# leoelm/Bayesian_inference_for_NN

Measured on AMD Instinct MI355X. Metric: posterior samples/sec (grad-steps/sec) on MLP 784->200->10, batch 1024, higher is better.
Workload: dtype f32; 1 GPU; SGLD, MLP 784->200->10 (D=159010), synthetic MNIST-shaped 48000x784 fp32 resident in HBM, batch 1024 (last batch of an epoch 896), 1 chain per GPU, device-resident run replayed from hipGraphs; seed=2024, parallelism=independent chains x1 (replicas only, no data-path collective)

## Files before the change

bayesian_inference_for_nn_amd/csrc/pyz_api.hip:

```cpp

#include <algorithm>
#include <cmath>
#include <cstring>

#include "pyz_common.h"
#include "pyz_fused.h"
#include "pyz_gemm.h"
#include "pyz_gemm_ring.h"
#include "pyz_hmc_fused.h"
#include "pyz_hmc_multi.h"
#include "pyz_kernels.h"
#include "pyz_rng.h"

namespace {

inline hipStream_t as_stream(void *s) { return reinterpret_cast<hipStream_t>(s); }
inline int cdiv(long long a, long long b) { return (int)((a + b - 1) / b); }

int ensure_bytes(void **ptr, size_t *cap, size_t need, pyz_mlp *m) {
  if (*cap >= need) return PYZ_OK;
  if (*ptr) PYZ_HIP(hipFree(*ptr));
  *ptr = nullptr;
  *cap = 0;
  PYZ_HIP(hipMalloc(ptr, need));
// ... 189 lines not shown
      g.out_pstride = (long long)m->max_batch * K;
      g.aux = m->act[l - 1];
      g.aux_pstride = (long long)m->max_batch * K;
      g.act = m->acts[l - 1];
      g.vec = (N % 8 == 0) && (m->w_off[l] % 4 == 0) && (P == 1 || theta_ps % 4 == 0) && aligned16(theta) ? 1 : 0;
      g.ctl = ctl;
      pyz_launch_bwd_data(g, grid_batch, P, st);
    }
    DenseArgs g{};
    g.K = K;
    g.N = N;
    if (l == 0) {
      g.in = x;
      g.in_pstride = 0;
      g.row_idx = row_idx;
    } else {
      g.in = m->act[l - 1];
      g.in_pstride = (long long)m->max_batch * K;
    }
    g.lda = K;
    g.aux = m->delta[l];
    g.aux_pstride = (long long)m->max_batch * N;
    g.out = grad;
    g.out_pstride = m->D;
    g.w_off = m->w_off[l];
    g.ctl = ctl;
    if (grad_sq) pyz_launch_bwd_weight_sq(g, grad_sq, grid_batch, st);
    else pyz_launch_bwd_weight(g, grid_batch, P, st);
  }
}

inline bool can_fuse(const pyz_mlp *m) { return m->dims[m->L] <= 32; }

void launch_head(pyz_mlp *m, const float *theta, long long theta_ps, int P, const float *x, const void *y,
                 const int32_t *row_idx, int grid_batch, const StepCtl *ctl, bool want_delta, hipStream_t st,
                 const StepCtl *gate = nullptr, int gate_mod = 0, int k_split = 0) {
  const int l = m->L - 1;
  HeadArgs g{};
  g.gate = gate;
  g.gate_mod = gate_mod;
  if (k_split > 1) {
    g.hparts = static_cast<const float *>(full(m)->x.fwd_part);
    g.n_hparts = k_split;
    g.hpart_stride = (long long)m->max_batch * m->dims[l];
    g.bias_prev = theta + m->w_off[l - 1] + (long long)m->dims[l - 1] * m->dims[l];
    g.h_store = m->act[l - 1];
  }
  g.K = m->dims[l];
  g.N = m->dims[l + 1];
  if (l == 0) {
    g.hin = x;
    g.hin_pstride = 0;
    g.gather_hin = 1;
  } else {
    g.hin = m->act[l - 1];
    g.hin_pstride = (long long)m->max_batch * g.K;
    g.gather_hin = 0;
  }
  g.lda = g.K;
  g.row_idx = row_idx;
  g.theta = theta;
  g.theta_pstride = theta_ps;
  g.w_off = m->w_off[l];
  g.loss = m->loss;
  g.act_last = m->acts[l];
  g.act_prev = l > 0 ? m->acts[l - 1] : PYZ_ACT_LINEAR;
  g.vec = (g.K % 8 == 0) && aligned16(g.hin) ? 1 : 0;
  g.y = y;
  g.out_last = m->act[l];
  g.delta_last = want_delta ? m->delta[l] : nullptr;
  g.delta_prev = (want_delta && l > 0) ? m->delta[l - 1] : nullptr;
  g.last_pstride = (long long)m->max_batch * g.N;
  g.prev_pstride = (long long)m->max_batch * g.K;
  g.part = m->part;
  g.ctl = ctl;
  g.wt = pyz_wt_for(P);
  if (m->pend_on && ctl == m->ctl) {
    g.init = m->pend;
    g.init_on = 1;
    m->pend_on = false;
  }
  static const int rows_on = pyz_env_int("PYZ_HEAD_ROWS", 1);
  const int UT = g.K <= 64 ? 1 : g.K <= 256 ? 4 : g.K <= 512 ? 8 : g.K <= 1024 ? 16 : 0;
  const int NP = g.N <= 4 ? 4 : g.N <= 8 ? 8 : g.N <= 12 ? 12 : g.N <= 16 ? 16 : g.N <= 24 ? 24 : 32;
  if (rows_on && UT && UT * NP <= 128) {
    g.nblk = grid_batch;
    m->cur_nblk = g.nblk;
    static const int rw_rows = pyz_env_int("PYZ_HEAD_RW_ROWS", 32768);
    const int RW = (long long)P * grid_batch >= rw_rows ? 4 : 1;
    const dim3 grid((unsigned)cdiv(cdiv(grid_batch, RW), 4), P), block(256);
    if (g.n_hparts > 0) {
      if (NP == 4) PYZ_LAUNCH((k_head_rows<4, 4, 1, true>), grid, block, 0, st, g);
      else if (NP == 8) PYZ_LAUNCH((k_head_rows<4, 8, 1, true>), grid, block, 0, st, g);
      else if (NP == 12) PYZ_LAUNCH((k_head_rows<4, 12, 1, true>), grid, block, 0, st, g);
      else PYZ_LAUNCH((k_head_rows<4, 16, 1, true>), grid, block, 0, st, g);
      return;
    }
#define PYZ_HEAD_ROWS_CASE(U, C)                                                               \
  if (UT == U && NP == C) {                                                                    \
    if (RW == 4) PYZ_LAUNCH((k_head_rows<U, C, 4>), grid, block, 0, st, g);                     \
    else PYZ_LAUNCH((k_head_rows<U, C, 1>), grid, block, 0, st, g);                            \
    return;                                                                                    \
  }
    PYZ_HEAD_ROWS_CASE(1, 4) PYZ_HEAD_ROWS_CASE(1, 8) PYZ_HEAD_ROWS_CASE(1, 12) PYZ_HEAD_ROWS_CASE(1, 16)
    PYZ_HEAD_ROWS_CASE(1, 24) PYZ_HEAD_ROWS_CASE(1, 32)
    PYZ_HEAD_ROWS_CASE(4, 4) PYZ_HEAD_ROWS_CASE(4, 8) PYZ_HEAD_ROWS_CASE(4, 12) PYZ_HEAD_ROWS_CASE(4, 16)
    PYZ_HEAD_ROWS_CASE(4, 24) PYZ_HEAD_ROWS_CASE(4, 32)
    PYZ_HEAD_ROWS_CASE(8, 4) PYZ_HEAD_ROWS_CASE(8, 8) PYZ_HEAD_ROWS_CASE(8, 12) PYZ_HEAD_ROWS_CASE(8, 16)
    PYZ_HEAD_ROWS_CASE(16, 4) PYZ_HEAD_ROWS_CASE(16, 8)
#undef PYZ_HEAD_ROWS_CASE
  }
  g.nblk = cdiv(grid_batch, 32);
  m->cur_nblk = g.nblk;
  static const int head_waves = pyz_env_int("PYZ_HEAD_WAVES", 8) >= 8 ? 8 : 4;
  PYZ_LAUNCH(k_head, dim3(g.nblk, P), dim3(64 * head_waves), head_waves * 4096 + 2 * 32 * 33 * 4 + 64, st, g);
}

void launch_bwd_data_hidden(pyz_mlp *m, const float *theta, long long theta_ps, int P, int grid_batch,
                            const StepCtl *ctl, hipStream_t st) {
  for (int l = m->L - 2; l >= 1; --l) {
    const int K = m->dims[l], N = m->dims[l + 1];
    DenseArgs g{};
    g.K = K;
    g.N = N;
    g.in = m->delta[l];
    g.in_pstride = (long long)m->max_batch * N;
    g.lda = N;
    g.theta = theta;
    g.theta_pstride = theta_ps;
    g.w_off = m->w_off[l];
    g.out = m->delta[l - 1];
    g.out_pstride = (long long)m->max_batch * K;
    g.aux = m->act[l - 1];
    g.aux_pstride = (long long)m->max_batch * K;
    g.act = m->acts[l - 1];
    g.vec = (N % 8 == 0) && (m->w_off[l] % 4 == 0) && (P == 1 || theta_ps % 4 == 0) && aligned16(theta) ? 1 : 0;
    g.ctl = ctl;
    pyz_launch_bwd_data(g, grid_batch, P, st);
  }
}

inline int wgrad_tiles(const pyz_mlp *m) {
  int tiles = 0;
  for (int l = 0; l < m->L; ++l) tiles += ((m->dims[l] + 1 + 31) / 32) * ((m->dims[l + 1] + 31) / 32);
  return tiles;
}

int wgrad_layers(pyz_mlp *m, int P, const float *x, const int32_t *row_idx, const StepCtl *ctl, WgradArgs &a,
// ... 68 lines not shown
  static const int on = pyz_env_int("PYZ_BATCH_AHEAD", 1);
  if (!on || !can_fuse(m) || m->L <= 1 || row_idx == nullptr) return false;
  return on == 2 || wgrad_tiles(m) + 24 <= pyz_cu_count();
}

PrepArgs prep_args(pyz_mlp *m, const float *x, const int32_t *row_idx, int grid_batch, long long row_stride, int dst_slot) {
  PrepArgs p{};
  p.src = x;
  p.dst = batch_buf(m, dst_slot);
  p.row_idx = row_idx;
  p.tab_bs = m->tab_bs;
  p.row_stride = row_stride;
  p.K = p.lda = m->dims[0];
  p.fwd_tiles_n = (m->dims[1] + 31) / 32;
  p.fwd_tiles = ((grid_batch + 31) / 32) * p.fwd_tiles_n;
  return p;
}

int ksplit_for(pyz_mlp *m, const float *theta, long long theta_ps, int P, const float *xc, int grid_batch, const StepCtl *ctl) {
  const int ks_env = pyz_env_int("PYZ_FWD_KSPLIT", 0);
  if (ks_env < 2 || ks_env > 8 || m->L != 2 || P != 1) return 0;
  const int UT = m->dims[1] <= 64 ? 1 : m->dims[1] <= 256 ? 4 : 0, NPc = m->dims[2];
  if (!UT || NPc > 16 || !pyz_env_int("PYZ_HEAD_ROWS", 1)) return 0;
  DenseArgs g = forward_args(m, 0, theta, theta_ps, xc, nullptr, ctl, nullptr);
  if (!pyz_fwd_ring_ksplit_ok(g, grid_batch, P)) return 0;
  if ((long long)((grid_batch + 31) / 32) * ks_env > 2 * pyz_cu_count()) return 0;
  const size_t need = sizeof(float) * (size_t)ks_env * m->max_batch * m->dims[1];
  if (!full(m)->x.fwd_part || full(m)->x.fwd_part_cap < need) return 0;
  return ks_env;
}

void launch_loss_backward(pyz_mlp *m, const float *theta, long long theta_ps, int P, const float *x, const void *y,
                          const int32_t *row_idx, int grid_batch, const StepCtl *ctl, bool want_grad, WgradArgs &upd,
                          hipStream_t st, int ahead_slot = -1, AdamArgs *adam = nullptr) {
  if (can_fuse(m)) {
    if (ahead_slot >= 0) {
      const float *xc = batch_buf(m, ahead_slot);
      const int ks = ksplit_for(m, theta, theta_ps, P, xc, grid_batch, ctl);
      if (ks > 1) {
        DenseArgs g = forward_args(m, 0, theta, theta_ps, xc, nullptr, ctl, nullptr);
        g.wt = pyz_wt_for(P);
        g.k_split = ks;
        g.part_out = static_cast<float *>(full(m)->x.fwd_part);
        g.part_stride = (long long)m->max_batch * g.N;
        pyz_launch_fwd_ring_ksplit(g, grid_batch, st);
      } else {
        launch_forward(m, theta, theta_ps, P, xc, nullptr, grid_batch, ctl, st, nullptr, m->L - 1);
      }
      launch_head(m, theta, theta_ps, P, x, y, row_idx, grid_batch, ctl, want_grad, st, nullptr, 0, ks);
      launch_bwd_data_hidden(m, theta, theta_ps, P, grid_batch, ctl, st);
      launch_wgrad_all(m, P, x, row_idx, grid_batch, ctl, upd, st, xc);
      return;
    }
    static const int use_xb = pyz_env_int("PYZ_GATHER_COPY", 1);
    float *xb = (use_xb && want_grad && row_idx && m->L > 1) ? m->xb : nullptr;
    launch_forward(m, theta, theta_ps, P, x, row_idx, grid_batch, ctl, st, xb, m->L - 1);
    launch_head(m, theta, theta_ps, P, x, y, row_idx, grid_batch, ctl, want_grad, st);
    if (want_grad) {
      launch_bwd_data_hidden(m, theta, theta_ps, P, grid_batch, ctl, st);
      if (adam) launch_wgrad_adam(m, x, row_idx, grid_batch, ctl, *adam, st, xb);
      else launch_wgrad_all(m, P, x, row_idx, grid_batch, ctl, upd, st, xb);
    }
    return;
  }
  flush_ctl(m, st);
  launch_forward(m, theta, theta_ps, P, x, row_idx, grid_batch, ctl, st);
  launch_loss(m, P, y, row_idx, grid_batch, ctl, want_grad, st);
  m->cur_nblk = loss_nblk(m, grid_batch);
  if (want_grad) launch_backward(m, theta, theta_ps, P, x, row_idx, grid_batch, ctl, upd.grad, st, adam ? m->grad2 : nullptr);
}

int check_loss_combo(const pyz_mlp *m) {
  const int last = m->acts[m->L - 1];
  if (m->loss == PYZ_LOSS_SCCE && last != PYZ_ACT_SOFTMAX)
    return pyz_fail(PYZ_E_INVALID, "SparseCategoricalCrossentropy needs a softmax last layer");
  if (m->loss == PYZ_LOSS_MSE && last == PYZ_ACT_SOFTMAX)
    return pyz_fail(PYZ_E_INVALID, "MeanSquaredError on a softmax last layer is not supported");
  return PYZ_OK;
}

AdamScal adam_scalars(float lr, double beta_1, double beta_2, long long epoch, float denom_eps, float decay) {
  AdamScal a;
// ... 61 lines not shown
    long long widest = 0;
    for (int l = 0; l <= n_layers; ++l) widest = std::max<long long>(widest, m->dims[l]);
    if ((long long)max_batch * widest * 4 >= (1LL << 31) || off * 4 >= (1LL << 31)) {
      delete m;
      return pyz_fail(PYZ_E_INVALID, "max_batch x widest layer, or the parameter vector, exceeds 2 GiB");
    }
  }
  auto fail = [&](int rc) {
    pyz_mlp_destroy(m);
    return rc;
  };
  for (int l = 0; l < n_layers; ++l) {
    const size_t bytes = sizeof(float) * (size_t)max_particles * max_batch * m->dims[l + 1] + 64;
    if (hipMalloc((void **)&m->act[l], bytes) != hipSuccess || hipMalloc((void **)&m->delta[l], bytes) != hipSuccess)
      return fail(pyz_fail(PYZ_E_OOM, "workspace allocation of %zu bytes failed", bytes));
    m->ws_bytes += 2 * bytes;
  }
  {
    const size_t bytes = 2 * sizeof(float) * (size_t)max_batch * m->dims[0] + 64;
    if (hipMalloc((void **)&m->xb, bytes) != hipSuccess) return fail(pyz_fail(PYZ_E_OOM, "workspace allocation of %zu bytes failed", bytes));
    m->ws_bytes += bytes;
  }
  if (hipMalloc((void **)&m->nonfinite, 64) != hipSuccess || hipMemset(m->nonfinite, 0, 64) != hipSuccess)
    return fail(pyz_fail(PYZ_E_OOM, "counter allocation failed"));
  if (hipMalloc((void **)&m->ctl, 2 * sizeof(StepCtl)) != hipSuccess) return fail(pyz_fail(PYZ_E_OOM, "ctl allocation failed"));
  if (hipMemset(m->ctl, 0, 2 * sizeof(StepCtl)) != hipSuccess) return fail(pyz_fail(PYZ_E_HIP, "ctl memset failed"));
  const size_t scal = sizeof(float) * (size_t)(max_particles * 16 + 64);
  if (hipMalloc((void **)&m->scal, scal) != hipSuccess) return fail(pyz_fail(PYZ_E_OOM, "scalar allocation failed"));
  m->ws_bytes += scal;
  {
    const int rc = need_part(m, (size_t)max_particles * max_batch + 8);
    if (rc != PYZ_OK) return fail(rc);
  }
  if (m->L == 2 && m->dims[1] > 192 && m->dims[1] <= 200 && pyz_env_int("PYZ_FWD_KSPLIT", 0) >= 2) {
    const int rc = ensure_bytes(&m->x.fwd_part, &m->x.fwd_part_cap, sizeof(float) * (size_t)8 * max_batch * m->dims[1], m);
    if (rc != PYZ_OK) return fail(rc);
  }
  {
    const int gs_lds = (int)pyz_svgd_gs_lds_bytes();
    if (hipFuncSetAttribute(reinterpret_cast<const void *>(k_svgd_gs<false>), hipFuncAttributeMaxDynamicSharedMemorySize, gs_lds) != hipSuccess ||
        hipFuncSetAttribute(reinterpret_cast<const void *>(k_svgd_gs<true>), hipFuncAttributeMaxDynamicSharedMemorySize, gs_lds) != hipSuccess)
      return fail(pyz_fail(PYZ_E_HIP, "hipFuncSetAttribute(k_svgd_gs) failed"));
    if (hipFuncSetAttribute(reinterpret_cast<const void *>(k_svgd_gs_resident), hipFuncAttributeMaxDynamicSharedMemorySize,
                            (int)pyz_svgd_gs_res_lds_bytes()) != hipSuccess)
      return fail(pyz_fail(PYZ_E_HIP, "hipFuncSetAttribute(k_svgd_gs_resident) failed"));
    if (hipFuncSetAttribute(reinterpret_cast<const void *>(k_svgd_gs_resident2), hipFuncAttributeMaxDynamicSharedMemorySize,
                            (int)pyz_svgd_gs_res_lds_bytes()) != hipSuccess)
      return fail(pyz_fail(PYZ_E_HIP, "hipFuncSetAttribute(k_svgd_gs_resident2) failed"));
    const int gr_lds = (int)pyz_svgd_gram_lds_bytes();
    if (hipFuncSetAttribute(reinterpret_cast<const void *>(k_svgd_gram_tile<1, false>), hipFuncAttributeMaxDynamicSharedMemorySize, gr_lds) != hipSuccess ||
        hipFuncSetAttribute(reinterpret_cast<const void *>(k_svgd_gram_tile<2, false>), hipFuncAttributeMaxDynamicSharedMemorySize, gr_lds) != hipSuccess ||
        hipFuncSetAttribute(reinterpret_cast<const void *>(k_svgd_gram_tile<4, true>), hipFuncAttributeMaxDynamicSharedMemorySize, gr_lds) != hipSuccess)
      return fail(pyz_fail(PYZ_E_HIP, "hipFuncSetAttribute(k_svgd_gram_tile) failed"));
  }
  *out = m;
  return PYZ_OK;
}

int pyz_mlp_destroy(pyz_mlp *mm) {
  if (!mm) return PYZ_OK;
  pyz_mlp_full *m = full(mm);
  drop_graphs(m);
  if (m->x.hm_exec) (void)hipGraphExecDestroy(m->x.hm_exec);
  if (m->x.hm_graph) (void)hipGraphDestroy(m->x.hm_graph);
  for (int l = 0; l < PYZ_MAX_LAYERS; ++l) {
    if (m->act[l]) (void)hipFree(m->act[l]);
    if (m->delta[l]) (void)hipFree(m->delta[l]);
  }
  void *ptrs[] = {m->grad, m->grad2, m->qsave, m->part, m->x.part2, m->scal, m->ctl, m->tab_bs, m->xb, m->x.hm_buf, m->x.hm_res_buf, m->x.gs_res_buf, m->x.fwd_part, m->nonfinite};
  for (void *p : ptrs)
    if (p) (void)hipFree(p);
  if (m->x.tab_host) {
    (void)hipHostFree(m->x.tab_host);
    for (auto &e : m->x.tab_ev) (void)hipEventDestroy(e);
  }
  if (m->x.up_host) {
    (void)hipHostFree(m->x.up_host);
    for (auto &e : m->x.up_ev) (void)hipEventDestroy(e);
  }
  if (m->h_pinned) (void)hipHostFree(m->h_pinned);
  delete m;
  return PYZ_OK;
}

int64_t pyz_mlp_param_count(const pyz_mlp *m) { return m ? m->D : -1; }
int64_t pyz_mlp_workspace_bytes(const pyz_mlp *m) { return m ? (int64_t)m->ws_bytes : -1; }

int pyz_mlp_forward(pyz_mlp *m, const float *d_theta, int P, const float *d_x, const int32_t *d_row_idx, int batch,
                    float *d_out, void *stream) {
  int rc = check_call(m, P, batch);
  if (rc) return rc;
  if (!d_theta || !d_x || !d_out) return pyz_fail(PYZ_E_INVALID, "null device pointer");
  hipStream_t st = as_stream(stream);
  if ((rc = set_ctl(m, 0, batch, 0.0f, 0, 0, 0, st))) return rc;
  launch_forward(m, d_theta, m->D, P, d_x, d_row_idx, batch, m->ctl, st);
  const int C = m->dims[m->L];
  PYZ_LAUNCH(k_forward_finish, dim3(cdiv(batch, 256), P), dim3(256), 0, st, m->act[m->L - 1],
                     (long long)m->max_batch * C, C, m->acts[m->L - 1] == PYZ_ACT_SOFTMAX ? 1 : 0, batch, d_out);
  PYZ_LAUNCH_CHECK();
  return PYZ_OK;
}

// ... 197 lines not shown
    const bool ahead = chained && batch_ahead(m, row_idx);
    if (ahead) u.prep = prep_args(m, x, row_idx, grid_batch, row_stride, slot ^ 1);
    launch_loss_backward(m, w_cur, m->D, 1, x, y, row_idx, grid_batch, ctl, true, u, st, ahead ? slot : -1);
    if (bbb->val) {
      pyz_mlp *v = bbb->val;
      launch_forward(v, w_cur, v->D, 1, bbb->val_x, nullptr, bbb->n_val, v->ctl, st, nullptr, v->L - 1, ctl, 10);
      launch_head(v, w_cur, v->D, 1, bbb->val_x, bbb->val_y, nullptr, bbb->n_val, v->ctl, false, st, ctl, 10);
      PYZ_LAUNCH(k_loss_finalize_gated, dim3(1), dim3(64), 0, st, v->part, v->cur_nblk, v->ctl, bbb->val_losses, v->nonfinite, ctl, 10);
    }
    return;
  }
  if (can_fuse(m)) {
    WgradArgs u{};
    u.mode = mode;
    if (swag) {
      u.swag_freq = swag->freq;
      u.swag_k = swag->k;
      u.dev_base = swag->dev;
      u.dev_stride = m->D;
    }
    u.theta = theta;
    u.mean = mean;
    u.sq_mean = sq;
    u.seed = seed;
    u.unit_noise = unit_noise;
    u.loss = loss;
    u.loss_indexed = chained ? 1 : 0;
    u.next = chained ? m->ctl + (slot ^ 1) : nullptr;
    u.tab_bs = m->tab_bs;
    u.tab_lr = m->tab_lr;
    u.row_stride = row_stride;
    const bool ahead = chained && batch_ahead(m, row_idx);
    if (ahead) u.prep = prep_args(m, x, row_idx, grid_batch, row_stride, slot ^ 1);
    launch_loss_backward(m, theta, m->D, 1, x, y, row_idx, grid_batch, ctl, true, u, st, ahead ? slot : -1);
    return;
  }
  WgradArgs u{};
  u.mode = PYZ_UPD_NONE;
  u.grad = m->grad;
  u.grad_pstride = m->D;
  launch_loss_backward(m, theta, m->D, 1, x, y, row_idx, grid_batch, ctl, true, u, st);
  SgldArgs a{};
  a.theta = theta;
  a.mean = mean;
  a.sq_mean = sq;
  a.grad = m->grad;
  a.D = m->D;
  a.ctl = ctl;
  a.next = chained ? m->ctl + (slot ^ 1) : nullptr;
  a.tab_bs = m->tab_bs;
  a.tab_lr = m->tab_lr;
  a.row_stride = row_stride;
  a.seed = seed;
  a.unit_noise = unit_noise;
  a.part = m->part;
  a.nblk = m->cur_nblk;
  a.loss = loss;
  a.loss_indexed = chained ? 1 : 0;
  a.nonfinite = m->nonfinite;
  PYZ_LAUNCH(k_sgld_update, dim3(cdiv(cdiv(m->D, 4), 256)), dim3(256), 0, st, a);
}

int pyz_sgld_step(pyz_mlp *m, float *d_theta, float *d_mean, float *d_sq_mean, const float *d_x, const void *d_y,
                  const int32_t *d_row_idx, int batch, float lr, int64_t n, uint64_t seed, const float *d_unit_noise,
                  float *d_loss, void *stream) {
  int rc = check_call(m, 1, batch);
  if (rc) return rc;
// ... 56 lines not shown
    m->tab_lr = nullptr;
    PYZ_HIP(hipMalloc((void **)&m->tab_bs, 8 * cap));
    m->tab_lr = reinterpret_cast<float *>(m->tab_bs + cap);
    m->tab_cap = (int)cap;
    drop_graphs(m);
  }
  if (f->x.tab_host_cap < 8 * n_tab) {
    if (f->x.tab_host) {
      PYZ_HIP(hipStreamSynchronize(st));
      PYZ_HIP(hipHostFree(f->x.tab_host));
      f->x.tab_host = nullptr;
    } else {
      for (auto &e : f->x.tab_ev) PYZ_HIP(hipEventCreateWithFlags(&e, hipEventDisableTiming));
    }
    const size_t cap = std::max<size_t>(8 * n_tab, 8 * 4096);
    PYZ_HIP(hipHostMalloc(&f->x.tab_host, 2 * cap));
    f->x.tab_host_cap = cap;
    f->x.tab_count = 0;
  }
  const long long row_stride = m->max_batch;
  bool first_batch_done = false;
  if (n_steps <= PYZ_INLINE_TAB) {
    InlineTabs tabs{};
    for (int s = 0; s < n_steps; ++s) {
      tabs.bs[s] = h_batch_sizes[s];
      tabs.lr[s] = h_lr[s];
    }
    tabs.bs[n_steps] = h_batch_sizes[n_steps - 1];
    tabs.lr[n_steps] = h_lr[n_steps - 1];
    tabs.n = n_steps + 1;
    m->pend_on = false;
    if (batch_ahead(m, d_row_idx)) {
      PYZ_LAUNCH(k_run_start, dim3(256), dim3(256), 0, st, m->ctl, tabs, m->tab_bs, m->tab_lr, (long long)n0, slot0 * row_stride,
                 (int)slot0, prep_args(m, d_x, d_row_idx, bmax, row_stride, 0));
      first_batch_done = true;
    } else {
      PYZ_LAUNCH(k_set_ctl_tabs, dim3(1), dim3(64), 0, st, m->ctl, tabs, m->tab_bs, m->tab_lr, (long long)n0, slot0 * row_stride, (int)slot0);
    }
  } else {
    const unsigned slot = (unsigned)(f->x.tab_count & 1);
    if (f->x.tab_count >= 2) PYZ_HIP(hipEventSynchronize(f->x.tab_ev[slot]));
    ++f->x.tab_count;
    int32_t *hb = reinterpret_cast<int32_t *>(static_cast<unsigned char *>(f->x.tab_host) + slot * f->x.tab_host_cap);
    float *hl = reinterpret_cast<float *>(hb + n_tab);
    std::memcpy(hb, h_batch_sizes, sizeof(int32_t) * n_steps);
    std::memcpy(hl, h_lr, sizeof(float) * n_steps);
    hb[n_steps] = h_batch_sizes[n_steps - 1];
    hl[n_steps] = h_lr[n_steps - 1];
    PYZ_HIP(hipMemcpyAsync(m->tab_bs, hb, sizeof(int32_t) * n_tab, hipMemcpyHostToDevice, st));
    PYZ_HIP(hipMemcpyAsync(m->tab_lr, hl, sizeof(float) * n_tab, hipMemcpyHostToDevice, st));
    PYZ_HIP(hipEventRecord(f->x.tab_ev[slot], st));
    if ((rc = set_ctl(m, 0, h_batch_sizes[0], h_lr[0], n0, slot0 * row_stride, 0, st, (int)slot0, n_steps))) return rc;
  }

  if (batch_ahead(m, d_row_idx) && !first_batch_done)
    PYZ_LAUNCH(k_prep_batch, dim3(256), dim3(256), 0, st, prep_args(m, d_x, d_row_idx, bmax, row_stride, 0), m->ctl);

  int s = 0;
  m->run_graph_steps = m->run_eager_steps = m->run_graph_launches = 0;
  static const int G = std::min(128, std::max(2, pyz_env_int("PYZ_GRAPH_STEPS", 32) & ~1));
  if (use_graph && st != nullptr && !pyz_probe().on) {
    unsigned long long key = 1469598103934665603ull;
    auto mix = [&](unsigned long long v) { key = (key ^ v) * 1099511628211ull; };
    mix((unsigned long long)(uintptr_t)d_theta); mix((unsigned long long)(uintptr_t)d_mean);
    mix((unsigned long long)(uintptr_t)d_sq_mean); mix((unsigned long long)(uintptr_t)d_x);
    mix((unsigned long long)(uintptr_t)d_y); mix((unsigned long long)(uintptr_t)d_row_idx);
    mix((unsigned long long)(uintptr_t)d_losses); mix(seed); mix((unsigned long long)bmax);
    mix((unsigned long long)(uintptr_t)m->tab_bs); mix((unsigned long long)G); mix((unsigned long long)mode);
    if (swag) { mix((unsigned long long)(uintptr_t)swag->dev); mix((unsigned long long)swag->k); mix((unsigned long long)swag->freq); }
    if (bbb) {
      unsigned fb[3];
      memcpy(&fb[0], &bbb->alpha, 4); memcpy(&fb[1], &bbb->prior_mean, 4); memcpy(&fb[2], &bbb->prior_rho, 4);
      for (unsigned b : fb) mix(b);
      mix((unsigned long long)(uintptr_t)bbb->pm_vec); mix((unsigned long long)(uintptr_t)bbb->pr_vec);
      mix((unsigned long long)(uintptr_t)bbb->val); mix((unsigned long long)(uintptr_t)bbb->val_x); mix((unsigned long long)(uintptr_t)bbb->val_y);
      mix((unsigned long long)bbb->n_val); mix((unsigned long long)(uintptr_t)bbb->val_losses);
      mix((unsigned long long)(uintptr_t)bbb->w2); mix((unsigned long long)(uintptr_t)bbb->rho); mix((unsigned long long)(uintptr_t)full(m)->x.part2);
    }
    if (m->graph_key != key) {
      drop_graphs(m);
      m->graph_key = key;
    }
    while (s < n_steps) {
      const int len = std::min(G, n_steps - s);
      int ci = 0;
      if (len < G) {
        ci = -1;
        int free_slot = -1, lru = -1;
        for (int c = 1; c < PYZ_GRAPH_CHUNKS; ++c) {
          if (!m->graph_exec[c]) {
            if (free_slot < 0) free_slot = c;
            continue;
          }
          if (m->graph_len[c] == len) ci = c;
          if (lru < 0 || m->graph_use[c] < m->graph_use[lru]) lru = c;
        }
        if (ci < 0) {
          ci = free_slot >= 0 ? free_slot : lru;
          if (m->graph_exec[ci]) (void)hipGraphExecDestroy(m->graph_exec[ci]);
          if (m->graph[ci]) (void)hipGraphDestroy(m->graph[ci]);
          m->graph_exec[ci] = nullptr;
// ... 985 lines not shown
```

bayesian_inference_for_nn_amd/csrc/pyz_common.h:

```cpp
#pragma once

#include <hip/hip_runtime.h>
#include <hip/hip_ext.h>

#include <cstdarg>
#include <cstdint>
#include <cstdio>
#include <string>
#include <vector>

#include "../../include/pyz.h"

#define PYZ_MAX_LAYERS 16

typedef float f32x16 __attribute__((ext_vector_type(16)));
typedef float f32x4 __attribute__((ext_vector_type(4)));

struct StepCtl {
  int32_t batch;
  float lr;
  long long n;
  long long row_off;
  int32_t i;
  int32_t slot0;
// ... 113 lines not shown
struct pyz_mlp {
  int L = 0;
  int dims[PYZ_MAX_LAYERS + 1] = {0};
  int acts[PYZ_MAX_LAYERS] = {0};
  long long w_off[PYZ_MAX_LAYERS] = {0};
  int loss = 0;
  int max_batch = 0, max_p = 0;
  long long D = 0;
  size_t ws_bytes = 0;
  float *act[PYZ_MAX_LAYERS] = {nullptr};
  float *delta[PYZ_MAX_LAYERS] = {nullptr};
  float *xb = nullptr;
  float *grad = nullptr;
  float *grad2 = nullptr;
  float *qsave = nullptr;
  double *part = nullptr;
  int part_len = 0;
  int cur_nblk = 0;
  float *scal = nullptr;
  StepCtl *ctl = nullptr;
  StepCtl pend{};
  bool pend_on = false;
  int32_t *tab_bs = nullptr;
  float *tab_lr = nullptr;
  int tab_cap = 0;
  float *h_pinned = nullptr;
  hipGraph_t graph[PYZ_GRAPH_CHUNKS] = {nullptr};
  hipGraphExec_t graph_exec[PYZ_GRAPH_CHUNKS] = {nullptr};
  int graph_len[PYZ_GRAPH_CHUNKS] = {0};
  unsigned long long graph_use[PYZ_GRAPH_CHUNKS] = {0}, graph_clock = 0;
  unsigned long long graph_key = 0;
  int run_graph_steps = 0, run_eager_steps = 0, run_graph_launches = 0;
  int *nonfinite = nullptr;
  int grad_owner = 0;
  int grad_rows = 0;
  bool km_valid = false;
  const float *km_all = nullptr;
  int km_total = 0, km_row0 = 0, km_local = 0;
  float km_gamma = 0.0f;
};
```

bayesian_inference_for_nn_amd/csrc/pyz_fused.h:

```cpp
#pragma once

#include "pyz_common.h"
#include "pyz_gemm.h"
#include "pyz_kernels.h"

struct HeadArgs {
  const float *hin;
  long long hin_pstride;
  int lda;
  const int32_t *row_idx;
  int gather_hin;
  const float *theta;
  long long theta_pstride;
  long long w_off;
  int K, N;
  int loss, act_last, act_prev, vec;
  const void *y;
  float *out_last;
  float *delta_last;
  float *delta_prev;
  long long last_pstride, prev_pstride;
  double *part;
  int nblk;
  const StepCtl *ctl;
// ... 207 lines not shown
  return v;
}

__device__ __forceinline__ float pyz_row16_allmax(float v) {
  v = fmaxf(v, pyz_dpp<0xB1>(v));
  v = fmaxf(v, pyz_dpp<0x4E>(v));
  v = fmaxf(v, pyz_dpp<0x141>(v));
  v = fmaxf(v, pyz_dpp<0x140>(v));
  return v;
}

template <int UT, int NP>
struct PyzHeadW {
  float wv[UT][NP];
  float bias_mine;
};

template <int UT, int NP>
__device__ __forceinline__ void pyz_head_load_w(const HeadArgs &g, const int p, const int l, PyzHeadW<UT, NP> &W) {
  const int K = g.K, N = g.N;
  const float *wl = g.theta + p * g.theta_pstride + g.w_off;
  const __amdgpu_buffer_rsrc_t rw = __builtin_amdgcn_make_buffer_rsrc(const_cast<float *>(wl), 0, (K + 1) * N * 4, 0x00020000);
  constexpr unsigned OOB = 0x7FFFFF00u;
#pragma unroll
  for (int t = 0; t < UT; ++t) {
    const int u = l + 64 * t;
    const unsigned wo = u < K ? 4u * (unsigned)u * (unsigned)N : OOB;
#pragma unroll
    for (int c = 0; c < NP; ++c) W.wv[t][c] = pyz_buf_load(rw, wo + 4u * (unsigned)c, 0u);
  }
  W.bias_mine = pyz_buf_load(rw, l < N ? 4u * ((unsigned)K * (unsigned)N + (unsigned)l) : OOB, 0u);
}

template <int UT, int NP, bool PRELOADED, bool HP = false>
__device__ __forceinline__ void pyz_head_row(const HeadArgs &g, const int batch, const long long row_off, const int p,
                                             const int m, const int l, PyzHeadW<UT, NP> &W) {
  const int K = g.K, N = g.N;
  long long yrow = m;
  if (g.row_idx) yrow = g.row_idx[row_off + m];
  const float *hp = g.hin + p * g.hin_pstride + (g.gather_hin ? yrow : (long long)m) * g.lda;
  const __amdgpu_buffer_rsrc_t rh = __builtin_amdgcn_make_buffer_rsrc(const_cast<float *>(hp), 0, K * 4, 0x00020000);
  float hv[UT], z[NP];
  if constexpr (HP) {
    const float *pp = g.hparts + (long long)m * K;
    const __amdgpu_buffer_rsrc_t rp = __builtin_amdgcn_make_buffer_rsrc(const_cast<float *>(pp), 0,
        (int)(((long long)(g.n_hparts - 1) * g.hpart_stride + K) * 4), 0x00020000);
    const __amdgpu_buffer_rsrc_t rb = __builtin_amdgcn_make_buffer_rsrc(const_cast<float *>(g.bias_prev), 0, K * 4, 0x00020000);
    constexpr unsigned OOBH = 0x7FFFFF00u;
    float pv[UT][8], bv[UT];
#pragma unroll
    for (int t = 0; t < UT; ++t) {
      const int u = l + 64 * t;
#pragma unroll
      for (int sp = 0; sp < 8; ++sp)
        pv[t][sp] = pyz_buf_load(rp, (u < K && sp < g.n_hparts) ? 4u * (unsigned)(sp * g.hpart_stride + u) : OOBH, 0u);
      bv[t] = pyz_buf_load(rb, 4u * (unsigned)u, 0u);
    }
#pragma unroll
    for (int t = 0; t < UT; ++t) {
      float a = pv[t][0];
#pragma unroll
      for (int sp = 1; sp < 8; ++sp) a += pv[t][sp];
      hv[t] = pyz_act(a + bv[t], g.act_prev);
      const int u = l + 64 * t;
      if (u < K) pyz_st(g.h_store + (long long)m * K + u, hv[t], g.wt);
    }
  } else {
#pragma unroll
    for (int t = 0; t < UT; ++t) hv[t] = pyz_buf_load(rh, 4u * (unsigned)(l + 64 * t), 0u);
  }
  if (!PRELOADED) pyz_head_load_w<UT, NP>(g, p, l, W);
  const auto &wv = W.wv;
  const float bias_mine = W.bias_mine;
  int ylab = 0;
  if (g.loss == PYZ_LOSS_SCCE) ylab = reinterpret_cast<const int32_t *>(g.y)[yrow];
  PYZ_STAMP(1, 1);
#pragma unroll
  for (int c = 0; c < NP; ++c) {
    float a = 0.0f;
#pragma unroll
    for (int t = 0; t < UT; ++t) a = fmaf(hv[t], wv[t][c], a);
    z[c] = a;
  }
#pragma unroll
  for (int c = 0; c < NP; ++c) {
    const float v = pyz_row16_allsum(z[c]);
    z[c] = ((pyz_readlane(v, 0) + pyz_readlane(v, 16)) + (pyz_readlane(v, 32) + pyz_readlane(v, 48))) + pyz_readlane(bias_mine, c);
  }
  PYZ_STAMP(1, 2);
  float d2[NP], lm, my_d = 0.0f, my_o = 0.0f;
  if (g.loss == PYZ_LOSS_SCCE && NP <= 16) {
    const int lc = l & 15;
    float zc = z[0];
#pragma unroll
    for (int c = 1; c < NP; ++c) zc = (lc == c) ? z[c] : zc;
    const bool on = lc < N;
    const float mx = pyz_row16_allmax(on ? zc : -3.0e38f);
    const float exv = on ? expf(zc - mx) : 0.0f;
    const float se = pyz_row16_allsum(exv);
    const float lse = mx + logf(se);
    const bool mine = on && lc == ylab;
    float zy = pyz_row16_allsum(mine ? zc : 0.0f);
// ... 64 lines not shown
#pragma unroll
    for (int c = 0; c < NP; ++c) a = fmaf(d2[c], wv[t][c], a);
    if (u < K) pyz_st(op + u, a * pyz_act_grad(hv[t], actp), g.wt);
  }
  PYZ_STAMP(1, 5);
}

template <int UT, int NP, int RW = 1, bool HP = false>
__global__ void __launch_bounds__(256) k_head_rows(HeadArgs g) {
  PYZ_STAMP(1, 0);
  const int w = pyz_wave_id(), l = threadIdx.x & 63;
  if (g.gate && g.gate->n % g.gate_mod == 0) return;
  const StepCtl ctl = pyz_ctl_first(g.ctl, g.init, g.init_on);
  const int batch = ctl.batch, p = blockIdx.y;
  const int m0 = (blockIdx.x * 4 + w) * RW;
  if (m0 >= batch) {
    if (l < RW && m0 + l < g.nblk) g.part[p * g.nblk + m0 + l] = 0.0;
    return;
  }
  PyzHeadW<UT, NP> W;
  if (RW == 1) {
    pyz_head_row<UT, NP, false, HP>(g, batch, ctl.row_off, p, m0, l, W);
    return;
  }
  pyz_head_load_w<UT, NP>(g, p, l, W);
#pragma unroll 1
  for (int rr = 0; rr < RW; ++rr) {
    const int m = m0 + rr;
    if (m >= batch) {
      if (l == 0 && m < g.nblk) g.part[p * g.nblk + m] = 0.0;
      continue;
    }
    pyz_head_row<UT, NP, true>(g, batch, ctl.row_off, p, m, l, W);
  }
}

struct PrepArgs {
  const float *src;
  float *dst;
  const int32_t *row_idx;
  const int32_t *tab_bs;
  long long row_stride;
  int K, lda;
  int fwd_tiles, fwd_tiles_n;
};

__device__ __forceinline__ void pyz_copy_rows(const PrepArgs &g, const int32_t *idx, const int ra, const int rb) {
  const int K = g.K, nt = blockDim.x, t = threadIdx.x;
  if (ra >= rb) return;
  if ((K & 3) == 0 && (g.lda & 3) == 0 && ((reinterpret_cast<uintptr_t>(g.src) | reinterpret_cast<uintptr_t>(g.dst)) & 15) == 0) {
    const int K4 = K >> 2, total = (rb - ra) * K4;
    for (int e0 = t; e0 < total; e0 += 4 * nt) {
      float4 v[4];
#pragma unroll
      for (int u = 0; u < 4; ++u) {
        const int e = min(e0 + u * nt, total - 1), m = ra + e / K4, c = e % K4;
        v[u] = *reinterpret_cast<const float4 *>(g.src + (long long)idx[m] * g.lda + 4 * c);
      }
#pragma unroll
      for (int u = 0; u < 4; ++u) {
        const int e = e0 + u * nt;
        if (e < total) {
          float *d = g.dst + (long long)(ra + e / K4) * K + 4 * (e % K4);
          const f32x4 vv = {v[u].x, v[u].y, v[u].z, v[u].w};
          asm volatile("global_store_dwordx4 %0, %1, off sc1" ::"v"(d), "v"(vv) : "memory");
        }
      }
    }
    return;
  }
  const int total = (rb - ra) * K;
  for (int e = t; e < total; e += nt) {
    const int m = ra + e / K, c = e % K;
    g.dst[(long long)m * K + c] = g.src[(long long)idx[m] * g.lda + c];
  }
}

__device__ __forceinline__ void pyz_prep_rows(const PrepArgs &g, const int32_t *idx, const int nb, const int j, const int cnt,
                                              const int bid) {
  int ra, rb;
  if (cnt >= 8 && g.fwd_tiles >= 8) {
    const int x = bid & 7, q = g.fwd_tiles >> 3, r = g.fwd_tiles & 7;
    const int t0 = x < r ? x * (q + 1) : r * (q + 1) + (x - r) * q, t1 = t0 + (x < r ? q + 1 : q);
    const int b0 = (t0 + g.fwd_tiles_n - 1) / g.fwd_tiles_n, b1 = (t1 + g.fwd_tiles_n - 1) / g.fwd_tiles_n;
    const int r0 = min(32 * b0, nb), r1 = x == 7 ? nb : min(32 * b1, nb);
    const int id0 = bid - j;
    const int first = id0 + ((x - (id0 & 7)) & 7);
    const int mine = (bid - first) >> 3, all = (id0 + cnt - 1 - first) / 8 + 1;
    const int per = (r1 - r0 + all - 1) / all;
    ra = r0 + mine * per;
    rb = min(ra + per, r1);
  } else {
    const int per = (nb + cnt - 1) / cnt;
    ra = j * per;
    rb = min(ra + per, nb);
  }
  pyz_copy_rows(g, idx, ra, rb);
}

__global__ void k_prep_batch(PrepArgs g, const StepCtl *ctl) {
  pyz_prep_rows(g, g.row_idx + ctl->row_off, ctl->batch, (int)blockIdx.x, (int)gridDim.x, (int)blockIdx.x);
}

__global__ void k_run_start(StepCtl *ctl, InlineTabs t, int32_t *tab_bs, float *tab_lr, long long n, long long row_off,
                            int slot0, PrepArgs g) {
  if (blockIdx.x == 0) {
    const int e = threadIdx.x;
    if (e < t.n) {
      tab_bs[e] = t.bs[e];
      tab_lr[e] = t.lr[e];
    }
    if (e == 0) {
      ctl->batch = t.bs[0];
      ctl->lr = t.lr[0];
      ctl->n = n;
      ctl->row_off = row_off;
      ctl->i = 0;
      ctl->slot0 = slot0;
      ctl->n_run = t.n - 1;
    }
  }
  pyz_prep_rows(g, g.row_idx + row_off, t.bs[0], (int)blockIdx.x, (int)gridDim.x, (int)blockIdx.x);
}

struct WgradLayer {
  const float *in;
  long long in_pstride;
  const float *delta;
  long long delta_pstride;
  long long w_off;
  int lda, K, N;
  int tile0;
  int gather;
};

#define PYZ_UPD_NONE 0
#define PYZ_UPD_SGD 1
#define PYZ_UPD_SGLD 2
#define PYZ_UPD_BBB 3
#define PYZ_UPD_SWAG 4

struct WgradArgs {
  WgradLayer lay[PYZ_MAX_LAYERS];
  int L;
  int tiles;
  const int32_t *row_idx;
  const StepCtl *ctl;
  int mode;
  float *grad;
  long long grad_pstride;
  float *theta, *mean, *sq_mean;
  uint64_t seed;
  const float *unit_noise;
  float *dev_row;
// ... 502 lines not shown
```

bayesian_inference_for_nn_amd/csrc/pyz_gemm.h:

```cpp
#pragma once

#include <cstdlib>

#include "pyz_common.h"

struct DenseArgs {
  const float *in;
  long long in_pstride;
  int lda;
  const float *theta;
  long long theta_pstride;
  long long w_off;
  int K, N;
  float *out;
  long long out_pstride;
  const float *aux;
  long long aux_pstride;
  int act;
  int vec;
  const StepCtl *ctl;
  const int32_t *row_idx;
  float *gather_out;
  StepCtl init;
  int init_on;
// ... 238 lines not shown
  long long row_off = 0;
  if (cap <= 0) {
    asm volatile("; the step scalars are needed here" ::: "memory");
    const StepCtl ctl = pyz_ctl_first(g.ctl, g.init, g.init_on);
    cap = __builtin_amdgcn_readfirstlane(ctl.batch);
    row_off = ctl.row_off;
  }
  if (m0 >= cap) return;
  const int p = blockIdx.y;
  const int K = g.K, N = g.N;
  const int m = min(m0 + r, cap - 1), n = min(n0 + r, N - 1);
  long long row = m;
  if (g.row_idx) row = g.row_idx[row_off + m];
  const float *ap = g.in + p * g.in_pstride + row * g.lda;
  const float *wl = g.theta + p * g.theta_pstride + g.w_off;
  f32x16 acc = {0};
  PYZ_STAMP(0, 1);
  float *gp = (g.gather_out && p == 0) ? g.gather_out + (long long)m * K : nullptr;
  int batch = 0;
  const int32_t *ctl_batch = &g.ctl->batch;
  pyz_fwd_accumulate(acc, ap, wl, n, K, N, g.vec, w, S, h, gp, tiles_n, tile % tiles_n,
                     [&]() { batch = __hip_atomic_load(ctl_batch, __ATOMIC_RELAXED, __HIP_MEMORY_SCOPE_AGENT); });
  batch = g.rows_cap > 0 ? __builtin_amdgcn_readfirstlane(batch) : cap;
  PYZ_STAMP(0, 2);
  float *op = g.out + p * g.out_pstride;
  const int act = g.act, wt = g.wt;
  pyz_tile_epilogue(acc, red, [&](int ro, int co, float v) {
    const int mm = m0 + ro, nn = n0 + co;
    if (mm < batch && nn < N) pyz_st(op + (long long)mm * N + nn, pyz_act(v, act), wt);
  });
  PYZ_STAMP(0, 3);
}

template <int NT>
__global__ void __launch_bounds__(256) k_dense_fwd_lds(DenseArgs g) {
  constexpr int BN = 32 * NT, BM = 128, BK = 16;
  constexpr int AS = BM + 32;
  constexpr int BS = (BN % 64 == 0) ? BN + 32 : BN;
  constexpr int BJ = NT;
  __shared__ __attribute__((aligned(16))) float As[2][BK][AS];
  __shared__ __attribute__((aligned(16))) float Bs[2][BK][BS];
  const int t = threadIdx.x, w = pyz_wave_id(), l = t & 63, r = l & 31, h = l >> 5;
  const StepCtl ctl = pyz_ctl_first(g.ctl, g.init, g.init_on);
  const int batch = ctl.batch;
  const int K = g.K, N = g.N;
  const int tiles_n = (N + BN - 1) / BN;
  const int tile = pyz_xcd_remap(blockIdx.x, gridDim.x);
  const int m0 = (tile / tiles_n) * BM, n0 = (tile % tiles_n) * BN;
  if (m0 >= batch) return;
  const int p = blockIdx.y;
  const int ra = t >> 1, ka = 8 * (t & 1);
  const int ma = min(m0 + ra, batch - 1);
  long long rowa = ma;
  if (g.row_idx) rowa = g.row_idx[ctl.row_off + ma];
  const float *ap = g.in + p * g.in_pstride + rowa * g.lda + ka;
  const float *wl = g.theta + p * g.theta_pstride + g.w_off;
  float *gp = (g.gather_out && p == 0 && n0 == 0 && m0 + ra < batch) ? g.gather_out + (long long)ma * K + ka : nullptr;
  float4 va[2];
  float2 vb[BJ];
  auto fetch = [&](const int k0) {
#pragma unroll
    for (int j = 0; j < 2; ++j) {
      const int k = k0 + ka + 4 * j;
      va[j] = k < K ? *reinterpret_cast<const float4 *>(ap + k0 + 4 * j) : make_float4(0.f, 0.f, 0.f, 0.f);
    }
#pragma unroll
// ... 335 lines not shown
```

Baseline: 40460 grad-steps/s.

## Fuse hidden-layer forward with loss head via per-row-tile ticket counters

Adds a fused kernel that computes the last hidden layer's forward tiles and, once every N-tile of a 32-row block has finished (tracked by an atomic ticket per row block), runs the loss/head computation in the last-arriving workgroup. This removes a separate head kernel launch and its dependency barrier in the SGLD step. The tickets are reset in the batch-prep kernels, and the head reads hidden activations with cache-coherent loads. The cost is a 1024-thread workgroup that does both stages, extra atomics, and serialization of the head on the last tile of each row block.

```diff
diff --git a/bayesian_inference_for_nn_amd/csrc/pyz_api.hip b/bayesian_inference_for_nn_amd/csrc/pyz_api.hip
--- a/bayesian_inference_for_nn_amd/csrc/pyz_api.hip
+++ b/bayesian_inference_for_nn_amd/csrc/pyz_api.hip
@@ -245,9 +245,8 @@
 
 inline bool can_fuse(const pyz_mlp *m) { return m->dims[m->L] <= 32; }
 
-void launch_head(pyz_mlp *m, const float *theta, long long theta_ps, int P, const float *x, const void *y,
-                 const int32_t *row_idx, int grid_batch, const StepCtl *ctl, bool want_delta, hipStream_t st,
-                 const StepCtl *gate = nullptr, int gate_mod = 0, int k_split = 0) {
+HeadArgs head_args(pyz_mlp *m, const float *theta, long long theta_ps, int P, const float *x, const void *y,
+                   const int32_t *row_idx, const StepCtl *ctl, bool want_delta, const StepCtl *gate, int gate_mod, int k_split) {
   const int l = m->L - 1;
   HeadArgs g{};
   g.gate = gate;
@@ -293,6 +292,13 @@
     g.init_on = 1;
     m->pend_on = false;
   }
+  return g;
+}
+
+void launch_head(pyz_mlp *m, const float *theta, long long theta_ps, int P, const float *x, const void *y,
+                 const int32_t *row_idx, int grid_batch, const StepCtl *ctl, bool want_delta, hipStream_t st,
+                 const StepCtl *gate = nullptr, int gate_mod = 0, int k_split = 0) {
+  HeadArgs g = head_args(m, theta, theta_ps, P, x, y, row_idx, ctl, want_delta, gate, gate_mod, k_split);
   static const int rows_on = pyz_env_int("PYZ_HEAD_ROWS", 1);
   const int UT = g.K <= 64 ? 1 : g.K <= 256 ? 4 : g.K <= 512 ? 8 : g.K <= 1024 ? 16 : 0;
   const int NP = g.N <= 4 ? 4 : g.N <= 8 ? 8 : g.N <= 12 ? 12 : g.N <= 16 ? 16 : g.N <= 24 ? 24 : 32;
@@ -327,6 +333,34 @@
   m->cur_nblk = g.nblk;
   static const int head_waves = pyz_env_int("PYZ_HEAD_WAVES", 8) >= 8 ? 8 : 4;
   PYZ_LAUNCH(k_head, dim3(g.nblk, P), dim3(64 * head_waves), head_waves * 4096 + 2 * 32 * 33 * 4 + 64, st, g);
+}
+
+bool launch_fwd_head(pyz_mlp *m, const float *theta, long long theta_ps, const float *xc, const float *x, const void *y,
+                     const int32_t *row_idx, int grid_batch, const StepCtl *ctl, hipStream_t st) {
+  if (!m->head_in_fwd || !m->tickets || m->L < 2 || !pyz_wt_for(1) || !pyz_env_int("PYZ_HEAD_ROWS", 1)) return false;
+  const int l = m->L - 2, K2 = m->dims[l + 1], N2 = m->dims[l + 2];
+  if (K2 > 256 || N2 > 16 || (K2 > 64 && N2 > 12) ||
+      grid_batch >= pyz_env_int("PYZ_HEAD_RW_ROWS", 32768)) return false;
+  DenseArgs g = forward_args(m, l, theta, theta_ps, xc, nullptr, ctl, nullptr);
+  if (g.init_on || g.row_idx) return false;
+  g.wt = 1;
+  g.rows_cap = std::min(grid_batch, m->max_batch);
+  const long long tiles = (long long)((grid_batch + 31) / 32) * ((g.N + 31) / 32);
+  const int S = pyz_pick_waves(tiles, (g.K + 1) / 2 + 1);
+  if (S != 16 || pyz_fwd_ring_variant(g, grid_batch, 1) || pyz_fwd_takes_lds(g, grid_batch, 1, S)) return false;
+  if ((grid_batch + 31) / 32 > m->n_tickets) return false;
+  launch_forward(m, theta, theta_ps, 1, xc, nullptr, grid_batch, ctl, st, nullptr, l);
+  HeadArgs h = head_args(m, theta, theta_ps, 1, x, y, row_idx, ctl, true, nullptr, 0, 0);
+  h.nblk = grid_batch;
+  m->cur_nblk = h.nblk;
+  const int UT = K2 <= 64 ? 1 : 4, NP = N2 <= 4 ? 4 : N2 <= 8 ? 8 : N2 <= 12 ? 12 : 16;
+  const dim3 grid((unsigned)tiles), block(1024);
+#define PYZ_FWD_HEAD_CASE(U, C) \
+  if (UT == U && NP == C) PYZ_LAUNCH((k_dense_fwd_head<U, C>), grid, block, 16 * 4096, st, g, h, m->tickets);
+  PYZ_FWD_HEAD_CASE(1, 4) PYZ_FWD_HEAD_CASE(1, 8) PYZ_FWD_HEAD_CASE(1, 12) PYZ_FWD_HEAD_CASE(1, 16)
+  PYZ_FWD_HEAD_CASE(4, 4) PYZ_FWD_HEAD_CASE(4, 8) PYZ_FWD_HEAD_CASE(4, 12)
+#undef PYZ_FWD_HEAD_CASE
+  return true;
 }
 
 void launch_bwd_data_hidden(pyz_mlp *m, const float *theta, long long theta_ps, int P, int grid_batch,
@@ -461,11 +495,13 @@
 
 void launch_loss_backward(pyz_mlp *m, const float *theta, long long theta_ps, int P, const float *x, const void *y,
                           const int32_t *row_idx, int grid_batch, const StepCtl *ctl, bool want_grad, WgradArgs &upd,
-                          hipStream_t st, int ahead_slot = -1, AdamArgs *adam = nullptr) {
+                          hipStream_t st, int ahead_slot = -1, AdamArgs *adam = nullptr, bool head_in_fwd = false) {
   if (can_fuse(m)) {
     if (ahead_slot >= 0) {
       const float *xc = batch_buf(m, ahead_slot);
       const int ks = ksplit_for(m, theta, theta_ps, P, xc, grid_batch, ctl);
+      const bool fused = ks <= 1 && head_in_fwd && P == 1 && want_grad &&
+                         launch_fwd_head(m, theta, theta_ps, xc, x, y, row_idx, grid_batch, ctl, st);
       if (ks > 1) {
         DenseArgs g = forward_args(m, 0, theta, theta_ps, xc, nullptr, ctl, nullptr);
         g.wt = pyz_wt_for(P);
@@ -473,10 +509,10 @@
         g.part_out = static_cast<float *>(full(m)->x.fwd_part);
         g.part_stride = (long long)m->max_batch * g.N;
         pyz_launch_fwd_ring_ksplit(g, grid_batch, st);
-      } else {
+      } else if (!fused) {
         launch_forward(m, theta, theta_ps, P, xc, nullptr, grid_batch, ctl, st, nullptr, m->L - 1);
       }
-      launch_head(m, theta, theta_ps, P, x, y, row_idx, grid_batch, ctl, want_grad, st, nullptr, 0, ks);
+      if (!fused) launch_head(m, theta, theta_ps, P, x, y, row_idx, grid_batch, ctl, want_grad, st, nullptr, 0, ks);
       launch_bwd_data_hidden(m, theta, theta_ps, P, grid_batch, ctl, st);
       launch_wgrad_all(m, P, x, row_idx, grid_batch, ctl, upd, st, xc);
       return;
@@ -604,6 +640,11 @@
     const int rc = need_part(m, (size_t)max_particles * max_batch + 8);
     if (rc != PYZ_OK) return fail(rc);
   }
+  m->head_in_fwd = pyz_env_int("PYZ_HEAD_IN_FWD", 1) != 0 ? 1 : 0;
+  m->n_tickets = (cdiv(max_batch, 32) + 3) / 4 * 4;
+  if (hipMalloc((void **)&m->tickets, sizeof(unsigned) * (size_t)m->n_tickets) != hipSuccess ||
+      hipMemset(m->tickets, 0, sizeof(unsigned) * (size_t)m->n_tickets) != hipSuccess)
+    return fail(pyz_fail(PYZ_E_OOM, "ticket allocation failed"));
   if (m->L == 2 && m->dims[1] > 192 && m->dims[1] <= 200 && pyz_env_int("PYZ_FWD_KSPLIT", 0) >= 2) {
     const int rc = ensure_bytes(&m->x.fwd_part, &m->x.fwd_part_cap, sizeof(float) * (size_t)8 * max_batch * m->dims[1], m);
     if (rc != PYZ_OK) return fail(rc);
@@ -639,7 +680,7 @@
     if (m->act[l]) (void)hipFree(m->act[l]);
     if (m->delta[l]) (void)hipFree(m->delta[l]);
   }
-  void *ptrs[] = {m->grad, m->grad2, m->qsave, m->part, m->x.part2, m->scal, m->ctl, m->tab_bs, m->xb, m->x.hm_buf, m->x.hm_res_buf, m->x.gs_res_buf, m->x.fwd_part, m->nonfinite};
+  void *ptrs[] = {m->grad, m->grad2, m->qsave, m->part, m->x.part2, m->scal, m->ctl, m->tab_bs, m->xb, m->x.hm_buf, m->x.hm_res_buf, m->x.gs_res_buf, m->x.fwd_part, m->nonfinite, m->tickets};
   for (void *p : ptrs)
     if (p) (void)hipFree(p);
   if (m->x.tab_host) {
@@ -903,7 +944,7 @@
     u.row_stride = row_stride;
     const bool ahead = chained && batch_ahead(m, row_idx);
     if (ahead) u.prep = prep_args(m, x, row_idx, grid_batch, row_stride, slot ^ 1);
-    launch_loss_backward(m, theta, m->D, 1, x, y, row_idx, grid_batch, ctl, true, u, st, ahead ? slot : -1);
+    launch_loss_backward(m, theta, m->D, 1, x, y, row_idx, grid_batch, ctl, true, u, st, ahead ? slot : -1, nullptr, ahead);
     return;
   }
   WgradArgs u{};
@@ -1026,7 +1067,7 @@
     m->pend_on = false;
     if (batch_ahead(m, d_row_idx)) {
       PYZ_LAUNCH(k_run_start, dim3(256), dim3(256), 0, st, m->ctl, tabs, m->tab_bs, m->tab_lr, (long long)n0, slot0 * row_stride,
-                 (int)slot0, prep_args(m, d_x, d_row_idx, bmax, row_stride, 0));
+                 (int)slot0, prep_args(m, d_x, d_row_idx, bmax, row_stride, 0), m->tickets, m->n_tickets);
       first_batch_done = true;
     } else {
       PYZ_LAUNCH(k_set_ctl_tabs, dim3(1), dim3(64), 0, st, m->ctl, tabs, m->tab_bs, m->tab_lr, (long long)n0, slot0 * row_stride, (int)slot0);
@@ -1048,7 +1089,7 @@
   }
 
   if (batch_ahead(m, d_row_idx) && !first_batch_done)
-    PYZ_LAUNCH(k_prep_batch, dim3(256), dim3(256), 0, st, prep_args(m, d_x, d_row_idx, bmax, row_stride, 0), m->ctl);
+    PYZ_LAUNCH(k_prep_batch, dim3(256), dim3(256), 0, st, prep_args(m, d_x, d_row_idx, bmax, row_stride, 0), m->ctl, m->tickets, m->n_tickets);
 
   int s = 0;
   m->run_graph_steps = m->run_eager_steps = m->run_graph_launches = 0;
@@ -1061,6 +1102,7 @@
     mix((unsigned long long)(uintptr_t)d_y); mix((unsigned long long)(uintptr_t)d_row_idx);
     mix((unsigned long long)(uintptr_t)d_losses); mix(seed); mix((unsigned long long)bmax);
     mix((unsigned long long)(uintptr_t)m->tab_bs); mix((unsigned long long)G); mix((unsigned long long)mode);
+    mix((unsigned long long)m->head_in_fwd);
     if (swag) { mix((unsigned long long)(uintptr_t)swag->dev); mix((unsigned long long)swag->k); mix((unsigned long long)swag->freq); }
     if (bbb) {
       unsigned fb[3];
diff --git a/bayesian_inference_for_nn_amd/csrc/pyz_common.h b/bayesian_inference_for_nn_amd/csrc/pyz_common.h
--- a/bayesian_inference_for_nn_amd/csrc/pyz_common.h
+++ b/bayesian_inference_for_nn_amd/csrc/pyz_common.h
@@ -169,6 +169,9 @@
   unsigned long long graph_key = 0;
   int run_graph_steps = 0, run_eager_steps = 0, run_graph_launches = 0;
   int *nonfinite = nullptr;
+  int head_in_fwd = 0;
+  unsigned *tickets = nullptr;
+  int n_tickets = 0;
   int grad_owner = 0;
   int grad_rows = 0;
   bool km_valid = false;
diff --git a/bayesian_inference_for_nn_amd/csrc/pyz_fused.h b/bayesian_inference_for_nn_amd/csrc/pyz_fused.h
--- a/bayesian_inference_for_nn_amd/csrc/pyz_fused.h
+++ b/bayesian_inference_for_nn_amd/csrc/pyz_fused.h
@@ -263,7 +263,11 @@
   W.bias_mine = pyz_buf_load(rw, l < N ? 4u * ((unsigned)K * (unsigned)N + (unsigned)l) : OOB, 0u);
 }
 
-template <int UT, int NP, bool PRELOADED, bool HP = false>
+__device__ __forceinline__ float pyz_buf_load_sc1(const __amdgpu_buffer_rsrc_t rsrc, const unsigned voff, const unsigned soff) {
+  return __builtin_bit_cast(float, __builtin_amdgcn_raw_buffer_load_b32(rsrc, (int)voff, (int)soff, 16));
+}
+
+template <int UT, int NP, bool PRELOADED, bool HP = false, bool SC1 = false>
 __device__ __forceinline__ void pyz_head_row(const HeadArgs &g, const int batch, const long long row_off, const int p,
                                              const int m, const int l, PyzHeadW<UT, NP> &W) {
   const int K = g.K, N = g.N;
@@ -298,7 +302,8 @@
     }
   } else {
 #pragma unroll
-    for (int t = 0; t < UT; ++t) hv[t] = pyz_buf_load(rh, 4u * (unsigned)(l + 64 * t), 0u);
+    for (int t = 0; t < UT; ++t)
+      hv[t] = SC1 ? pyz_buf_load_sc1(rh, 4u * (unsigned)(l + 64 * t), 0u) : pyz_buf_load(rh, 4u * (unsigned)(l + 64 * t), 0u);
   }
   if (!PRELOADED) pyz_head_load_w<UT, NP>(g, p, l, W);
   const auto &wv = W.wv;
@@ -429,6 +434,57 @@
       continue;
     }
     pyz_head_row<UT, NP, true>(g, batch, ctl.row_off, p, m, l, W);
+  }
+}
+
+template <int UT, int NP>
+__global__ void __launch_bounds__(1024) k_dense_fwd_head(DenseArgs g, HeadArgs hd, unsigned *tickets) {
+  extern __shared__ float red[];
+  constexpr int NPRE = ((64 * UT + 1) * NP + 1023) / 1024;
+  int m0, batch;
+  (void)pyz_dense_fwd_tile<16>(g, red, m0, batch);
+  const int w = pyz_wave_id(), l = threadIdx.x & 63;
+  const int K = hd.K, N = hd.N, tot = (K + 1) * N;
+  const float *wl = hd.theta + hd.w_off;
+  float wpre[NPRE];
+#pragma unroll
+  for (int i = 0; i < NPRE; ++i) wpre[i] = wl[min((int)threadIdx.x + 1024 * i, tot - 1)];
+  const long long row_off = hd.ctl->row_off;
+  asm volatile("s_waitcnt vmcnt(0)" ::: "memory");
+  __syncthreads();
+  if (threadIdx.x == 0) {
+    const unsigned tiles_n = (unsigned)((g.N + 31) >> 5);
+    const unsigned old = __hip_atomic_fetch_add(tickets + (m0 >> 5), 1u, __ATOMIC_RELAXED, __HIP_MEMORY_SCOPE_AGENT);
+    red[0] = (old + 1u) % tiles_n == 0u ? 1.0f : 0.0f;
+  }
+  __syncthreads();
+  if (red[0] == 0.0f) return;
+  PYZ_STAMP(1, 0);
+  float *wlds = red + 64;
+#pragma unroll
+  for (int i = 0; i < NPRE; ++i) {
+    const int e = (int)threadIdx.x + 1024 * i;
+    if (e < tot) wlds[e] = wpre[i];
+  }
+  __syncthreads();
+  PyzHeadW<UT, NP> W;
+#pragma unroll
+  for (int t = 0; t < UT; ++t) {
+    const int u = l + 64 * t;
+#pragma unroll
+    for (int c = 0; c < NP; ++c) {
+      const int e = u * N + c;
+      W.wv[t][c] = (u < K && e < tot) ? wlds[e] : 0.0f;
+    }
+  }
+  W.bias_mine = l < N ? wlds[K * N + l] : 0.0f;
+#pragma unroll 1
+  for (int m = m0 + w; m < m0 + 32; m += 16) {
+    if (m >= batch) {
+      if (l == 0 && m < hd.nblk) hd.part[m] = 0.0;
+      continue;
+    }
+    pyz_head_row<UT, NP, true, false, true>(hd, batch, row_off, 0, m, l, W);
   }
 }
 
@@ -495,12 +551,18 @@
   pyz_copy_rows(g, idx, ra, rb);
 }
 
-__global__ void k_prep_batch(PrepArgs g, const StepCtl *ctl) {
+__device__ __forceinline__ void pyz_zero_tickets(unsigned *tickets, const int n) {
+  if (tickets && blockIdx.x == gridDim.x - 1)
+    for (int i = threadIdx.x; i < n; i += blockDim.x) tickets[i] = 0u;
+}
+
+__global__ void k_prep_batch(PrepArgs g, const StepCtl *ctl, unsigned *tickets, int n_tickets) {
+  pyz_zero_tickets(tickets, n_tickets);
   pyz_prep_rows(g, g.row_idx + ctl->row_off, ctl->batch, (int)blockIdx.x, (int)gridDim.x, (int)blockIdx.x);
 }
 
 __global__ void k_run_start(StepCtl *ctl, InlineTabs t, int32_t *tab_bs, float *tab_lr, long long n, long long row_off,
-                            int slot0, PrepArgs g) {
+                            int slot0, PrepArgs g, unsigned *tickets, int n_tickets) {
   if (blockIdx.x == 0) {
     const int e = threadIdx.x;
     if (e < t.n) {
@@ -517,6 +579,7 @@
       ctl->n_run = t.n - 1;
     }
   }
+  pyz_zero_tickets(tickets, n_tickets);
   pyz_prep_rows(g, g.row_idx + row_off, t.bs[0], (int)blockIdx.x, (int)gridDim.x, (int)blockIdx.x);
 }
 
diff --git a/bayesian_inference_for_nn_amd/csrc/pyz_gemm.h b/bayesian_inference_for_nn_amd/csrc/pyz_gemm.h
--- a/bayesian_inference_for_nn_amd/csrc/pyz_gemm.h
+++ b/bayesian_inference_for_nn_amd/csrc/pyz_gemm.h
@@ -294,6 +294,69 @@
   PYZ_STAMP(0, 3);
 }
 
+template <int S, class F>
+__device__ __forceinline__ void pyz_tile_epilogue_fixed(const f32x16 &acc, float *red, F store) {
+  const int w = pyz_wave_id(), l = threadIdx.x & 63;
+  const int r = l & 31, h = l >> 5;
+  float *my = red + w * 1024;
+#pragma unroll
+  for (int i = 0; i < 16; ++i) my[((i & 3) + 8 * (i >> 2) + 4 * h) * 32 + r] = acc[i];
+  __syncthreads();
+  for (int e = threadIdx.x; e < 1024; e += 64 * S) {
+    float s = red[e];
+    for (int ww = 1; ww < S; ++ww) s += red[ww * 1024 + e];
+    store(e >> 5, e & 31, s);
+  }
+}
+
+template <int S>
+__device__ __forceinline__ bool pyz_dense_fwd_tile(const DenseArgs &g, float *red, int &m0, int &batch) {
+  PYZ_STAMP(0, 0);
+  const int w = pyz_wave_id(), l = threadIdx.x & 63;
+  const int r = l & 31, h = l >> 5;
+  const int tiles_n = (g.N + 31) >> 5;
+  m0 = batch = 0;
+  if (g.gate && g.gate->n % g.gate_mod == 0) return false;
+  const int tile = pyz_xcd_remap(blockIdx.x, gridDim.x);
+  const int n0 = (tile % tiles_n) * 32;
+  m0 = (tile / tiles_n) * 32;
+  int cap = g.rows_cap;
+  long long row_off = 0;
+  if (cap <= 0) {
+    asm volatile("; the step scalars are needed here" ::: "memory");
+    const StepCtl ctl = pyz_ctl_first(g.ctl, g.init, g.init_on);
+    cap = __builtin_amdgcn_readfirstlane(ctl.batch);
+    row_off = ctl.row_off;
+  }
+  batch = cap;
+  if (m0 >= cap) return false;
+  const int p = blockIdx.y;
+  const int K = g.K, N = g.N;
+  const int m = min(m0 + r, cap - 1), n = min(n0 + r, N - 1);
+  long long row = m;
+  if (g.row_idx) row = g.row_idx[row_off + m];
+  const float *ap = g.in + p * g.in_pstride + row * g.lda;
+  const float *wl = g.theta + p * g.theta_pstride + g.w_off;
+  f32x16 acc = {0};
+  PYZ_STAMP(0, 1);
+  float *gp = (g.gather_out && p == 0) ? g.gather_out + (long long)m * K : nullptr;
+  batch = 0;
+  const int32_t *ctl_batch = &g.ctl->batch;
+  pyz_fwd_accumulate(acc, ap, wl, n, K, N, g.vec, w, S, h, gp, tiles_n, tile % tiles_n,
+                     [&]() { batch = __hip_atomic_load(ctl_batch, __ATOMIC_RELAXED, __HIP_MEMORY_SCOPE_AGENT); });
+  batch = g.rows_cap > 0 ? __builtin_amdgcn_readfirstlane(batch) : cap;
+  PYZ_STAMP(0, 2);
+  float *op = g.out + p * g.out_pstride;
+  const int act = g.act, wt = g.wt;
+  const int rows = batch, row0 = m0;
+  pyz_tile_epilogue_fixed<S>(acc, red, [&, rows, row0](int ro, int co, float v) {
+    const int mm = row0 + ro, nn = n0 + co;
+    if (mm < rows && nn < N) pyz_st(op + (long long)mm * N + nn, pyz_act(v, act), wt);
+  });
+  PYZ_STAMP(0, 3);
+  return true;
+}
+
 template <int NT>
 __global__ void __launch_bounds__(256) k_dense_fwd_lds(DenseArgs g) {
   constexpr int BN = 32 * NT, BM = 128, BK = 16;
```

Result: slower. 32380 grad-steps/s (-20.0%).
